# geoeo/ORB_SLAM3_V1.0

Measured on AMD Instinct MI355X. Metric: frames/sec ORB extract+match, 752x480 8-level 1000-feat; bit-exact kp/desc, higher is better.
Workload: dtype u8

## Files before the change

orb_slam3_v1.0_amd/csrc/kernels_match_proj.hip:

```cpp
#include <algorithm>
#include <cstdio>
#include <cstdlib>
#include <cstring>

#include "device_math.h"
#include "match_common.h"

#include "match_proj.h"

#pragma clang fp contract(off)

namespace orbfe {

using namespace proj;

namespace {


template <bool LDS, class KeyFn>
__device__ __forceinline__ void block_sort_keys(unsigned long long* sKeys, unsigned long long* gKeys, int n, int P, int tid, KeyFn keyOf)
{
    for (int j = tid; j < P; j += 1024) {
        const unsigned long long key = j < n ? keyOf(j) : ~0ull;
        if constexpr (LDS) sKeys[j] = key;
        else gKeys[j] = key;
    }
    __syncthreads();
    for (int k2 = 2; k2 <= P; k2 <<= 1) {
        for (int j2 = k2 >> 1; j2 > 0; j2 >>= 1) {
            for (int t = tid; t < (P >> 1); t += 1024) {
                const int lo = ((t & ~(j2 - 1)) << 1) | (t & (j2 - 1));
                const int hi = lo | j2;
                const bool up = (lo & k2) == 0;
                unsigned long long a, b;
                if constexpr (LDS) { a = sKeys[lo]; b = sKeys[hi]; }
                else { a = gKeys[lo]; b = gKeys[hi]; }
                if ((a > b) == up) {
                    if constexpr (LDS) { sKeys[lo] = b; sKeys[hi] = a; }
                    else { gKeys[lo] = b; gKeys[hi] = a; }
                }
            }
            __syncthreads();
        }
    }
}

template <class KeyFn>
__device__ __forceinline__ void block_sort_keys_reg(unsigned long long* sKeys, int n, int P, int tid, KeyFn keyOf)
{
    unsigned long long key = tid < n ? keyOf(tid) : ~0ull;
    int buf = 0;
    for (int k2 = 2; k2 <= P; k2 <<= 1) {
        for (int j2 = k2 >> 1; j2 > 0; j2 >>= 1) {
            unsigned long long other;
            if (j2 >= 64) {
                unsigned long long* b = sKeys + buf * 1024;
                b[tid] = key;
                __syncthreads();
                other = b[tid ^ j2];
                buf ^= 1;
            } else {
                other = shfl_xor_u64(key, j2);
            }
            const bool up = (tid & k2) == 0;
            const bool lower = (tid & j2) == 0;
            const unsigned long long mn = key < other ? key : other, mx = key < other ? other : key;
            key = (lower == up) ? mn : mx;
        }
    }
    __syncthreads();
    sKeys[tid] = key;
    __syncthreads();
}

constexpr int kCellBits = 22;

template <bool LDS>
__device__ __forceinline__ void proj_grid_body(const ProjArgs& A)
{
    __shared__ unsigned long long sKeys[LDS ? kSortLds : 1];
    __shared__ int sRankOf[LDS ? kSortLds : 1];
    const int f = blockIdx.x;
    const int tid = threadIdx.x;
    const int n = min(A.nKp[f], A.kpStride);
    const int nCells = A.g.cols * A.g.rows;
    const orbfe_keypoint* kp = A.kp + (size_t)f * A.kpStride;
    unsigned long long* gKeys = A.sortKeys + (size_t)f * A.sortCap;
    int* gRankOf = A.rankOf + (size_t)f * A.kpStride;
    int P = 1;
    while (P < n) P <<= 1;
    for (int j = tid; j < A.kpStride; j += 1024) A.matchOut[(size_t)f * A.kpStride + j] = -1;
    auto cellOf = [&](int j) {
        const orbfe_keypoint& k = kp[j];
        float px = k.x - A.g.minX;
        px = px * A.g.invW;
        float py = k.y - A.g.minY;
        py = py * A.g.invH;
        const int posX = (int)roundf(px), posY = (int)roundf(py);
        const int lin = posY * A.g.cols + posX;
        int v = nCells;
        if (lin >= 0 && lin < nCells) v = (lin % A.g.cols) * A.g.rows + lin / A.g.cols;
        return v;
    };
    auto key1 = [&](int j) { return ((unsigned long long)cellOf(j) << kRankBits) | (unsigned long long)j; };
    const bool regSort = LDS && P <= 1024;
    if (regSort) block_sort_keys_reg(sKeys, n, P, tid, key1);
    else block_sort_keys<LDS>(sKeys, gKeys, n, P, tid, key1);
    for (int r = tid; r < n; r += 1024) {
        unsigned long long key;
        if constexpr (LDS) key = sKeys[r];
        else key = gKeys[r];
        const int idx = (int)(key & kRankMask);
        A.order[(size_t)f * A.kpStride + r] = idx;
        A.octByRank[(size_t)f * A.kpStride + r] = (uint8_t)min(max(kp[idx].octave, 0), 31);
        if constexpr (LDS) sRankOf[idx] = r;
        else gRankOf[idx] = r;
    }
    __syncthreads();
    auto key2 = [&](int j) {
        const unsigned long long lvl = (unsigned long long)min(max(kp[j].octave, 0), 31);
        return (lvl << (kRankBits + kCellBits + 1)) | ((unsigned long long)cellOf(j) << kRankBits) | (unsigned long long)j;
    };
    if (regSort) block_sort_keys_reg(sKeys, n, P, tid, key2);
    else block_sort_keys<LDS>(sKeys, gKeys, n, P, tid, key2);
    const unsigned long long* desc = reinterpret_cast<const unsigned long long*>(A.desc + (size_t)f * A.kpStride * 32);
    for (int p = tid; p < n; p += 1024) {
        unsigned long long key;
        if constexpr (LDS) key = sKeys[p];
        else key = gKeys[p];
        const int idx = (int)(key & kRankMask);
        const int v = (int)((key >> kRankBits) & ((1u << (kCellBits + 1)) - 1u));
        const int lvl = (int)(key >> (kRankBits + kCellBits + 1));
        const orbfe_keypoint k = kp[idx];
        int rank;
        if constexpr (LDS) rank = sRankOf[idx];
        else rank = gRankOf[idx];
        const int cy = v < nCells ? v % A.g.rows : 0x7fff;
        A.rec[(size_t)f * A.kpStride + p] = make_int4(rank, lvl | (cy << 8), __float_as_int(k.x), __float_as_int(k.y));
        unsigned long long* dd = A.descS + ((size_t)f * A.kpStride + p) * 4;
        dd[0] = desc[(size_t)idx * 4 + 0];
        dd[1] = desc[(size_t)idx * 4 + 1];
        dd[2] = desc[(size_t)idx * 4 + 2];
        dd[3] = desc[(size_t)idx * 4 + 3];
    }
    const int tabStride = A.g.cols + 1;
    int* cs = A.colStart + (size_t)f * A.tabLevels * tabStride;
    const int nTab = A.tabLevels * tabStride;
    for (int e = tid; e < nTab; e += 1024) {
        const int l = e / tabStride;
        const int v = (e - l * tabStride) * A.g.rows;
        const unsigned long long want = ((unsigned long long)l << (kCellBits + 1)) | (unsigned long long)v;
        int lo = 0, hi = n;
        while (lo < hi) {
            const int mid = (lo + hi) >> 1;
            unsigned long long key;
            if constexpr (LDS) key = sKeys[mid];
            else key = gKeys[mid];
            if ((key >> kRankBits) < want) lo = mid + 1;
            else hi = mid;
        }
        cs[e] = lo;
    }
}

constexpr int kTilesX = 8, kTilesY = 6;
constexpr int kSortBuckets = 32 * kTilesX * kTilesY + 1;

__device__ __forceinline__ int sort_bucket(const ProjArgs& A, const orbfe_map_point& mp)
{
    const bool valid = mp.in_view && !(A.farPoints && mp.track_depth > A.thFar) && !mp.bad;
    if (!valid) return kSortBuckets - 1;
    const int lvl = min(max(mp.level, 0), 31);
    const int cx = (int)((mp.proj_x - A.g.minX) * A.g.invW), cy = (int)((mp.proj_y - A.g.minY) * A.g.invH);
    const int tx = min(max(cx * kTilesX / A.g.cols, 0), kTilesX - 1);
    const int ty = min(max(cy * kTilesY / A.g.rows, 0), kTilesY - 1);
    return (lvl * kTilesY + ty) * kTilesX + tx;
}

__device__ __forceinline__ void proj_sort_body(const ProjArgs& A)
{
    __shared__ int sHist[kSortBuckets];
    const int f = blockIdx.x;
    const int tid = threadIdx.x;
    for (int b = tid; b < kSortBuckets; b += 1024) sHist[b] = 0;
    __syncthreads();
    const orbfe_map_point* mps = A.mps + (size_t)f * A.M;
    for (int i = tid; i < A.M; i += 1024) atomicAdd(&sHist[sort_bucket(A, mps[i])], 1);
    __syncthreads();
    {
        static_assert(kSortBuckets <= 2048, "two buckets per thread");
        __shared__ int sWaveTot[16];
        const int b0 = 2 * tid, b1 = 2 * tid + 1;
        const int c0 = b0 < kSortBuckets ? sHist[b0] : 0, c1 = b1 < kSortBuckets ? sHist[b1] : 0;
        const int lane = tid & 63, wv = tid >> 6;
        int incl = c0 + c1;
#pragma unroll
        for (int d = 1; d < 64; d <<= 1) {
            const int o = __shfl_up(incl, d);
            if (lane >= d) incl += o;
        }
        if (lane == 63) sWaveTot[wv] = incl;
        __syncthreads();
        int base = incl - (c0 + c1);
        for (int q = 0; q < wv; q++) base += sWaveTot[q];
        if (b0 < kSortBuckets) sHist[b0] = base;
        if (b1 < kSortBuckets) sHist[b1] = base + c0;
    }
    __syncthreads();
    for (int i = tid; i < A.M; i += 1024) {
        const int pos = atomicAdd(&sHist[sort_bucket(A, mps[i])], 1);
        A.perm[(size_t)f * A.M + pos] = i;
    }
}

template <bool LDS, bool SORT_MPS>
__global__ __launch_bounds__(1024) void proj_prepare_kernel(ProjArgs A)
{
    if constexpr (SORT_MPS) {
        if (blockIdx.y == 1) {
            proj_sort_body(A);
            return;
        }
    }
    proj_grid_body<LDS>(A);
}

constexpr int kTopkLds = 768;

struct TopkLds {
    int4 rec[kTopkLds];
    unsigned long long desc[kTopkLds][4];
};

__device__ __forceinline__ void topk_insert_round(uint32_t (&keys)[kTopK], uint32_t (&pend)[kTopkPend])
{
    const uint32_t key = pend[0];
#pragma unroll
    for (int t = 0; t < kTopkPend - 1; t++) pend[t] = pend[t + 1];
    pend[kTopkPend - 1] = kKey32None;
#pragma unroll
    for (int t = kTopK - 1; t > 0; t--) keys[t] = umed3(keys[t - 1], key, keys[t]);
    keys[0] = min(keys[0], key);
}

template <bool LDS, bool WIDE>
__device__ __forceinline__ int topk_scan(const ProjArgs& A, const MpWindow& w, const int* cs, int tabStride, const int4* rec,
                                         const unsigned long long* descS, const TopkLds* S, int segBase,
                                         unsigned long long d0, unsigned long long d1, unsigned long long d2,
                                         unsigned long long d3, uint32_t (&keys)[kTopK])
{
    int total = 0;
    uint32_t pend[kTopkPend];
#pragma unroll
    for (int t = 0; t < kTopkPend; t++) pend[t] = kKey32None;
    const int lFirst = max(w.minLevel, 0), l1 = w.maxLevel;
    for (int l0 = lFirst; l0 <= (WIDE ? l1 : lFirst); l0 += 2) {
    int plo[2], phi[2];
#pragma unroll
    for (int k = 0; k < 2; k++) {
        const int l = min(l0 + k, l1);
        const int* csl = cs + (size_t)l * tabStride;
        plo[k] = csl[w.minCX];
        phi[k] = (l0 + k <= l1) ? csl[w.maxCX + 1] : plo[k];
    }
#pragma unroll
    for (int k = 0; k < 2; k++) {
        int4 qn = make_int4(0, 0, 0, 0);
        if (plo[k] < phi[k]) {
            if constexpr (LDS) qn = S->rec[plo[k] - segBase];
            else qn = rec[plo[k]];
        }
        for (int p = plo[k]; p < phi[k]; p++) {
            const int4 q = qn;
            if (p + 1 < phi[k]) {
                if constexpr (LDS) qn = S->rec[p + 1 - segBase];
                else qn = rec[p + 1];
            }
            const int cy = q.y >> 8;
            const float dx = __int_as_float(q.z) - w.x, dy = __int_as_float(q.w) - w.y;
            if (cy >= w.minCY && cy <= w.maxCY && fabsf(dx) < w.r && fabsf(dy) < w.r) {
                int dist;
                if constexpr (LDS) {
                    const unsigned long long* kd = S->desc[p - segBase];
                    dist = hamming256(kd, d0, d1, d2, d3);
                } else {
                    const unsigned long long* kd = descS + (size_t)p * 4;
                    dist = hamming256(kd, d0, d1, d2, d3);
                }
                if (dist < A.dCut) {
                    total++;
                    const uint32_t key = make_key32(dist, q.x);
                    if (key < keys[kTopK - 1]) {
#pragma unroll
                        for (int t = kTopkPend - 1; t > 0; t--) pend[t] = pend[t - 1];
                        pend[0] = key;
                    }
                }
            }
            if (__ballot(pend[kTopkPend - 1] != kKey32None)) topk_insert_round(keys, pend);
        }
    }
    }
    while (__ballot(pend[0] != kKey32None)) topk_insert_round(keys, pend);
    return total;
}

template <bool WIDE>
__global__ __launch_bounds__(256) void proj_topk_kernel(ProjArgs A)
{
    __shared__ TopkLds S;
    __shared__ int sLvlLo, sLvlHi;
    const int f = blockIdx.y;
    const int slotIdx = blockIdx.x * 256 + threadIdx.x;
    const bool live = slotIdx < A.M;
    const int i = live ? A.perm[(size_t)f * A.M + slotIdx] : 0;
    MpWindow w;
    w.valid = false;
    w.minLevel = w.maxLevel = 0;
    if (live) w = mp_window(A, A.mps[(size_t)f * A.M + i]);
    if (threadIdx.x == 0) { sLvlLo = 64; sLvlHi = -1; }
    __syncthreads();
    if (w.valid) {
        atomicMin(&sLvlLo, max(w.minLevel, 0));
        atomicMax(&sLvlHi, w.maxLevel);
    }
    __syncthreads();
    const int tabStride = A.g.cols + 1;
    const int* cs = A.colStart + (size_t)f * A.tabLevels * tabStride;
    const int4* rec = A.rec + (size_t)f * A.kpStride;
    const unsigned long long* descS = A.descS + (size_t)f * A.kpStride * 4;
    int segBase = 0, segEnd = 0;
    if (sLvlHi >= 0) {
        segBase = cs[(size_t)sLvlLo * tabStride];
        segEnd = sLvlHi + 1 < A.tabLevels ? cs[(size_t)(sLvlHi + 1) * tabStride] : min(A.nKp[f], A.kpStride);
    }
    const bool useLds = segEnd - segBase <= kTopkLds;
    if (useLds) {
        const int nSeg = segEnd - segBase;
        const uint4* gRec = reinterpret_cast<const uint4*>(rec + segBase);
        const uint4* gDesc = reinterpret_cast<const uint4*>(descS + (size_t)segBase * 4);
        uint4* lRec = reinterpret_cast<uint4*>(S.rec);
        uint4* lDesc = reinterpret_cast<uint4*>(&S.desc[0][0]);
        for (int j0 = 0; j0 < nSeg * 2; j0 += 4 * 256) {
            uint4 v[4];
#pragma unroll
            for (int k = 0; k < 4; k++) {
                const int j = j0 + k * 256 + (int)threadIdx.x;
                v[k] = make_uint4(0u, 0u, 0u, 0u);
                if (j < nSeg * 2) v[k] = gDesc[j];
            }
#pragma unroll
            for (int k = 0; k < 4; k++) {
                const int j = j0 + k * 256 + (int)threadIdx.x;
                if (j < nSeg * 2) lDesc[j] = v[k];
            }
        }
        for (int j0 = 0; j0 < nSeg; j0 += 4 * 256) {
            uint4 v[4];
#pragma unroll
            for (int k = 0; k < 4; k++) {
                const int j = j0 + k * 256 + (int)threadIdx.x;
                v[k] = make_uint4(0u, 0u, 0u, 0u);
                if (j < nSeg) v[k] = gRec[j];
            }
#pragma unroll
            for (int k = 0; k < 4; k++) {
                const int j = j0 + k * 256 + (int)threadIdx.x;
                if (j < nSeg) lRec[j] = v[k];
            }
        }
    }
    __syncthreads();
    if (!live) return;
    uint32_t keys[kTopK];
#pragma unroll
    for (int t = 0; t < kTopK; t++) keys[t] = kKey32None;
    int total = 0;
    if (w.valid) {
        const unsigned long long* dp = reinterpret_cast<const unsigned long long*>(A.mpDesc + ((size_t)f * A.M + i) * 32);
        const unsigned long long d0 = dp[0], d1 = dp[1], d2 = dp[2], d3 = dp[3];
        if (useLds) total = topk_scan<true, WIDE>(A, w, cs, tabStride, rec, descS, &S, segBase, d0, d1, d2, d3, keys);
        else total = topk_scan<false, WIDE>(A, w, cs, tabStride, rec, descS, &S, segBase, d0, d1, d2, d3, keys);
    }
    A.cnt[(size_t)f * A.M + i] = total;
    uint4* dst = reinterpret_cast<uint4*>(A.topk + ((size_t)f * A.M + i) * kTopK);
#pragma unroll
    for (int t = 0; t < kTopK / 4; t++) dst[t] = make_uint4(keys[4 * t], keys[4 * t + 1], keys[4 * t + 2], keys[4 * t + 3]);
}

constexpr int kWaveListCap = 128;

__device__ __forceinline__ void rank_emit_lds(const uint32_t* list, int n, int limit, uint32_t* out, int lane)
{
    const uint32_t e0 = lane < n ? list[lane] : kKey32None;
    const uint32_t e1 = lane + 64 < n ? list[lane + 64] : kKey32None;
    int r0 = 0, r1 = 0;
    for (int b = 0; b < n; b++) {
        const uint32_t kb = list[b];
        r0 += kb < e0;
        r1 += kb < e1;
    }
    __builtin_amdgcn_wave_barrier();
    if (lane < n && r0 < limit) out[r0] = e0;
    if (lane + 64 < n && r1 < limit) out[r1] = e1;
    asm volatile("s_waitcnt lgkmcnt(0)" ::: "memory");
    __builtin_amdgcn_wave_barrier();
}

template <bool WIDE, bool LDS>
__device__ __forceinline__ void topk_wave_body(const ProjArgs& A, const TopkLds& S, uint32_t (*sList)[2][kWaveListCap], int f, int lane,
                                               int wv, int nMine, int i, const MpWindow& w, const int* cs, int tabStride,
                                               const int4* rec, const unsigned long long* descS, int segBase)
{
    constexpr int NLV = WIDE ? 3 : 2;
    int plo[NLV], phi[NLV];
    {
        const int l0 = max(w.minLevel, 0), l1 = w.maxLevel;
#pragma unroll
        for (int k = 0; k < NLV; k++) {
            const int l = min(l0 + k, l1);
            const int* csl = cs + (size_t)l * tabStride;
            plo[k] = w.valid ? csl[w.minCX] : 0;
            phi[k] = (w.valid && l0 + k <= l1) ? csl[w.maxCX + 1] : plo[k];
        }
    }
    const int validI = w.valid ? 1 : 0;
    uint32_t dq[8] = {0, 0, 0, 0, 0, 0, 0, 0};
    if (w.valid) {
        const uint4* dp = reinterpret_cast<const uint4*>(A.mpDesc + ((size_t)f * A.M + i) * 32);
        const uint4 a = dp[0], b = dp[1];
        dq[0] = a.x; dq[1] = a.y; dq[2] = a.z; dq[3] = a.w; dq[4] = b.x; dq[5] = b.y; dq[6] = b.z; dq[7] = b.w;
    }
#pragma unroll
    for (int k = 0; k < NLV; k++) asm volatile("" : "+v"(plo[k]), "+v"(phi[k]));
#pragma unroll
    for (int k = 0; k < 8; k++) asm volatile("" : "+v"(dq[k]));
    {
        int iv = i;
        asm volatile("s_waitcnt vmcnt(0)" : "+v"(iv));
    }
    for (int j = 0; j < nMine; j++) {
        const int mp = __builtin_amdgcn_readlane(i, j);
        uint32_t* dst = A.topk + ((size_t)f * A.M + mp) * kTopK;
        int total = 0, listN = 0, cur = 0;
        if (__builtin_amdgcn_readlane(validI, j)) {
            const float x = __int_as_float(__builtin_amdgcn_readlane(__float_as_int(w.x), j));
            const float y = __int_as_float(__builtin_amdgcn_readlane(__float_as_int(w.y), j));
            const float r = __int_as_float(__builtin_amdgcn_readlane(__float_as_int(w.r), j));
            const int minCY = __builtin_amdgcn_readlane(w.minCY, j), maxCY = __builtin_amdgcn_readlane(w.maxCY, j);
            unsigned long long d[4];
#pragma unroll
            for (int k = 0; k < 4; k++)
                d[k] = (unsigned long long)(uint32_t)__builtin_amdgcn_readlane((int)dq[2 * k], j) |
                       ((unsigned long long)(uint32_t)__builtin_amdgcn_readlane((int)dq[2 * k + 1], j) << 32);
            int a[NLV], len[NLV], lenAll = 0;
#pragma unroll
            for (int k = 0; k < NLV; k++) {
                a[k] = __builtin_amdgcn_readlane(plo[k], j);
                len[k] = __builtin_amdgcn_readlane(phi[k], j) - a[k];
                lenAll += len[k];
            }
            for (int base = 0; base < lenAll; base += 64) {
                if (listN > 64) {
                    rank_emit_lds(sList[wv][cur], listN, 64, sList[wv][cur ^ 1], lane);
                    cur ^= 1;
                    listN = 64;
                }
                const int idx = base + lane;
                bool q = false;
                uint32_t key = kKey32None;
                if (idx < lenAll) {
                    int p = a[0] + idx;
                    if (idx >= len[0]) p = a[1] + (idx - len[0]);
                    if constexpr (NLV == 3)
                        if (idx >= len[0] + len[1]) p = a[2] + (idx - len[0] - len[1]);
                    int4 rq;
                    if constexpr (LDS) rq = S.rec[p - segBase];
                    else rq = rec[p];
                    const int cy = rq.y >> 8;
                    const float dx = __int_as_float(rq.z) - x, dy = __int_as_float(rq.w) - y;
                    if (cy >= minCY && cy <= maxCY && fabsf(dx) < r && fabsf(dy) < r) {
                        int dist;
                        if constexpr (LDS) {
                            const unsigned long long* kd = S.desc[p - segBase];
                            dist = hamming256(kd, d[0], d[1], d[2], d[3]);
                        } else {
                            const unsigned long long* kd = descS + (size_t)p * 4;
                            dist = hamming256(kd, d[0], d[1], d[2], d[3]);
                        }
                        if (dist < A.dCut) {
                            q = true;
                            key = make_key32(dist, rq.x);
                        }
                    }
                }
                const unsigned long long mask = __ballot(q);
                if (mask) {
                    if (q)
                        sList[wv][cur][listN + (int)__builtin_amdgcn_mbcnt_hi((uint32_t)(mask >> 32),
                                                                              __builtin_amdgcn_mbcnt_lo((uint32_t)mask, 0u))] = key;
                    const int c = __popcll(mask);
                    listN += c;
                    total += c;
                }
            }
            if (total) {
                asm volatile("s_waitcnt lgkmcnt(0)" ::: "memory");
                __builtin_amdgcn_wave_barrier();
                if (listN > 64) {
                    rank_emit_lds(sList[wv][cur], listN, 64, sList[wv][cur ^ 1], lane);
                    cur ^= 1;
                    listN = 64;
                }
                const uint32_t e = lane < listN ? sList[wv][cur][lane] : kKey32None;
                int rk = 0;
                for (int b = 0; b < listN; b++) rk += (uint32_t)__builtin_amdgcn_readlane((int)e, b) < e;
                if (lane < listN && rk < kTopK) dst[rk] = e;
                if (lane >= listN && lane < kTopK) dst[lane] = kKey32None;
            }
        }
        if (lane == 0) A.cnt[(size_t)f * A.M + mp] = total;
    }
}

template <bool WIDE>
__global__ __launch_bounds__(256) void proj_topk_wave_kernel(ProjArgs A, int mpw)
{
    __shared__ TopkLds S;
    __shared__ int sLvlLo, sLvlHi;
    __shared__ uint32_t sList[4][2][kWaveListCap];
    const int f = blockIdx.y;
    const int lane = threadIdx.x & 63;
    const int wv = __builtin_amdgcn_readfirstlane((int)(threadIdx.x >> 6));
    const int waveBase = (blockIdx.x * 4 + wv) * mpw;
    const int nMine = min(mpw, A.M - waveBase);
    const bool live = lane < nMine;
    const int i = live ? A.perm[(size_t)f * A.M + waveBase + lane] : 0;
    MpWindow w;
    w.valid = false;
    w.minLevel = w.maxLevel = 0;
    w.x = w.y = w.r = 0.0f;
    w.minCX = w.maxCX = w.minCY = w.maxCY = 0;
    if (live) w = mp_window(A, A.mps[(size_t)f * A.M + i]);
    if (threadIdx.x == 0) { sLvlLo = 64; sLvlHi = -1; }
    __syncthreads();
    if (w.valid) {
        atomicMin(&sLvlLo, max(w.minLevel, 0));
        atomicMax(&sLvlHi, w.maxLevel);
    }
    __syncthreads();
    const int tabStride = A.g.cols + 1;
    const int* cs = A.colStart + (size_t)f * A.tabLevels * tabStride;
    const int4* rec = A.rec + (size_t)f * A.kpStride;
    const unsigned long long* descS = A.descS + (size_t)f * A.kpStride * 4;
    int segBase = 0, segEnd = 0;
    if (sLvlHi >= 0) {
        segBase = cs[(size_t)sLvlLo * tabStride];
        segEnd = sLvlHi + 1 < A.tabLevels ? cs[(size_t)(sLvlHi + 1) * tabStride] : min(A.nKp[f], A.kpStride);
    }
    const bool useLds = segEnd - segBase <= kTopkLds;
    if (useLds) {
        const int nSeg = segEnd - segBase;
        const uint4* gRec = reinterpret_cast<const uint4*>(rec + segBase);
        const uint4* gDesc = reinterpret_cast<const uint4*>(descS + (size_t)segBase * 4);
        uint4* lRec = reinterpret_cast<uint4*>(S.rec);
        uint4* lDesc = reinterpret_cast<uint4*>(&S.desc[0][0]);
        for (int j0 = 0; j0 < nSeg * 2; j0 += 4 * 256) {
            uint4 v[4];
#pragma unroll
            for (int k = 0; k < 4; k++) {
                const int j = j0 + k * 256 + (int)threadIdx.x;
                if (j < nSeg * 2) v[k] = gDesc[j];
            }
#pragma unroll
            for (int k = 0; k < 4; k++) {
                const int j = j0 + k * 256 + (int)threadIdx.x;
                if (j < nSeg * 2) lDesc[j] = v[k];
            }
        }
        for (int j0 = 0; j0 < nSeg; j0 += 4 * 256) {
            uint4 v[4];
#pragma unroll
            for (int k = 0; k < 4; k++) {
                const int j = j0 + k * 256 + (int)threadIdx.x;
                if (j < nSeg) v[k] = gRec[j];
            }
#pragma unroll
            for (int k = 0; k < 4; k++) {
                const int j = j0 + k * 256 + (int)threadIdx.x;
                if (j < nSeg) lRec[j] = v[k];
            }
        }
    }
    __syncthreads();
    if (useLds) topk_wave_body<WIDE, true>(A, S, sList, f, lane, wv, nMine, i, w, cs, tabStride, rec, descS, segBase);
    else topk_wave_body<WIDE, false>(A, S, sList, f, lane, wv, nMine, i, w, cs, tabStride, rec, descS, segBase);
}

constexpr int kResN = 2048;

constexpr int kResNDesc = 1280;

template <int N, bool DESC, bool IMG>
struct ResolveLdsT {
    int claim[3][N];
    uint8_t oct[IMG ? N : 1];
    int4 rec[IMG ? N : 1];
    unsigned long long desc[DESC ? N * 4 : 4];
};

template <bool IMG, bool DESC, typename SLds>
__device__ __forceinline__ void full_scan_top2_wave(const ProjArgs& A, int f, int i, const MpWindow& w,
                                                    const unsigned long long (&d4)[4], const int* cs, const int* claim,
                                                    const SLds* S, int lane, uint32_t& k1, uint32_t& k2)
{
    k1 = kKey32None;
    k2 = kKey32None;
    if (w.valid) {
        const int tabStride = A.g.cols + 1;
        const int4* rec = A.rec + (size_t)f * A.kpStride;
        const unsigned long long* descS = A.descS + (size_t)f * A.kpStride * 4;
        for (int l = max(w.minLevel, 0); l <= w.maxLevel; l++) {
            const int* csl = cs + (size_t)l * tabStride;
            const int plo = csl[w.minCX], phi = csl[w.maxCX + 1];
            for (int p = plo + lane; p < phi; p += 64) {
                int4 q;
                if constexpr (IMG) q = S->rec[p];
                else q = rec[p];
                if (claim[q.x] < i) continue;
                const int cy = q.y >> 8;
                if (cy < w.minCY || cy > w.maxCY) continue;
                const float dx = __int_as_float(q.z) - w.x, dy = __int_as_float(q.w) - w.y;
                if (!(fabsf(dx) < w.r && fabsf(dy) < w.r)) continue;
                int dist;
                if constexpr (DESC) dist = hamming256(reinterpret_cast<const uint2*>(S->desc + (size_t)p * 4), d4);
                else dist = hamming256(reinterpret_cast<const uint2*>(descS + (size_t)p * 4), d4);
                if (dist >= A.dCut) continue;
                const uint32_t key = make_key32(dist, q.x);
                k2 = umed3(k1, key, k2);
                k1 = min(k1, key);
            }
        }
    }
    wave_top2_u32(k1, k2);
}

constexpr int kFbLds = 192;
constexpr int kResTabLds = 1024;
constexpr int kFbBatched = 32;

template <bool LDS, int THREADS, int N = kResN, bool DESC = false, bool IMG = LDS, int FB = kFbLds>
__global__ __launch_bounds__(THREADS) void proj_resolve_kernel(ProjArgs A)
{
    static_assert(LDS || !IMG, "the LDS image goes with LDS claim tables");
    __shared__ ResolveLdsT<N, DESC, IMG> S;
    __shared__ int sChanged[2];
    __shared__ int sGaveUp[2];
    __shared__ int sCount;
    __shared__ int sFbCount[2];
    __shared__ int sFbMp[THREADS];
    __shared__ uint32_t sFbK1[THREADS], sFbK2[THREADS];
    __shared__ MpWindow sFbWin[FB];
    __shared__ unsigned long long sFbDesc[FB][4];
    __shared__ int sTab[LDS ? kResTabLds : 1];
    const int f = blockIdx.x;
    const int tid = threadIdx.x;
    const int n = min(A.nKp[f], A.kpStride);
    const int M = A.M;
    int* Tfin = LDS ? S.claim[0] : A.claimG + ((size_t)f * 3 + 0) * A.kpStride;
    int* Tcur = LDS ? S.claim[1] : A.claimG + ((size_t)f * 3 + 1) * A.kpStride;
    int* Tnxt = LDS ? S.claim[2] : A.claimG + ((size_t)f * 3 + 2) * A.kpStride;
    const orbfe_map_point* mps = A.mps + (size_t)f * M;
    const int* order = A.order + (size_t)f * A.kpStride;
    const int4* rec = A.rec + (size_t)f * A.kpStride;
    const int* initObs = A.initObs ? A.initObs + (size_t)f * A.kpStride : nullptr;

    for (int r = tid; r < n; r += THREADS) {
        const int v = (initObs && initObs[order[r]] > 0) ? -1 : kClaimFree;
        Tfin[r] = v;
        Tcur[r] = v;
    }
    const uint8_t* octByRank = A.octByRank + (size_t)f * A.kpStride;
    if constexpr (IMG) {
        for (int r = tid; r < n; r += THREADS) {
            S.rec[r] = rec[r];
            S.oct[r] = octByRank[r];
        }
    }
    if constexpr (DESC) {
        const unsigned long long* dsrc = A.descS + (size_t)f * A.kpStride * 4;
        for (int q = tid; q < n * 4; q += THREADS) S.desc[q] = dsrc[q];
    }
    const int tabStride = A.g.cols + 1;
    const int* csG = A.colStart + (size_t)f * A.tabLevels * tabStride;
    const bool tabInLds = LDS && A.tabLevels * tabStride <= kResTabLds;
    if (tabInLds)
        for (int k = tid; k < A.tabLevels * tabStride; k += THREADS) sTab[k] = csG[k];
    const int* cs = tabInLds ? sTab : csG;
    if (tid == 0) sCount = 0;
    int nAccepted = 0;
    __syncthreads();

    for (int chunk = 0; chunk < M; chunk += THREADS) {
        const int i = chunk + tid;
        const bool live = i < M;
        int c = 0, obs = 0;
        uint32_t keys[kTopK];
#pragma unroll
        for (int t = 0; t < kTopK; t++) keys[t] = kKey32None;
        if (live) {
            c = A.cnt[(size_t)f * M + i];
            obs = mps[i].observations;
            if (c > 0) {
                const uint4* src = reinterpret_cast<const uint4*>(A.topk + ((size_t)f * M + i) * kTopK);
#pragma unroll
                for (int t = 0; t < kTopK / 4; t++) {
                    const uint4 q = src[t];
                    keys[4 * t] = q.x; keys[4 * t + 1] = q.y; keys[4 * t + 2] = q.z; keys[4 * t + 3] = q.w;
                }
            }
        }
        int res = -1;
        uint32_t k1 = kKey32None, k2 = kKey32None;
        bool k2StandIn = false;
        for (int iter = 0; iter <= THREADS + 1; iter++) {
            if (tid == 0) { sChanged[iter & 1] = 0; sFbCount[iter & 1] = 0; sGaveUp[iter & 1] = 0; }
            if (res >= 0 && obs > 0) atomicMin(&Tcur[res], i);
            __syncthreads();
            const int* claim = Tcur;
            bool look = iter == 0 || sGaveUp[(iter & 1) ^ 1] != 0;
            if (!look && c > 0) {
                const int c1 = k1 != kKey32None ? claim[(int)(k1 & kRankMask)] : kClaimFree;
                const int c2 = (k2 != kKey32None && !k2StandIn) ? claim[(int)(k2 & kRankMask)] : kClaimFree;
                look = c1 < i || c2 < i;
            }
            int slot = -1;
            if (c > 0 && look) {
                k1 = kKey32None;
                k2 = kKey32None;
                k2StandIn = false;
                int cl[kTopK];
#pragma unroll
                for (int t = 0; t < kTopK; t++) cl[t] = claim[keys[t] != kKey32None ? (int)(keys[t] & kRankMask) : 0];
#pragma unroll
                for (int t = 0; t < kTopK; t++) {
                    const uint32_t m = cl[t] >= i ? keys[t] : kKey32None;
                    k2 = umed3(k1, m, k2);
                    k1 = min(k1, m);
                }
                if (k2 == kKey32None && c > kTopK) {
                    const int dK = (int)(keys[kTopK - 1] >> kRankBits);
                    bool decided = false;
                    if (k1 == kKey32None) decided = dK > ORBFE_TH_HIGH;
                    else {
                        const int bd = (int)(k1 >> kRankBits);
                        decided = bd > ORBFE_TH_HIGH || (A.nnRatio > 0.f && !((float)bd > A.nnRatio * (float)dK));
                        if (decided) {
                            k2 = keys[kTopK - 1];
                            k2StandIn = true;
                        }
                    }
                    if (!decided) {
                        slot = atomicAdd(&sFbCount[iter & 1], 1);
                        sFbMp[slot] = i;
                        if (slot < FB) {
                            sFbWin[slot] = mp_window(A, mps[i]);
                            const unsigned long long* dp = reinterpret_cast<const unsigned long long*>(A.mpDesc + ((size_t)f * M + i) * 32);
#pragma unroll
                            for (int t = 0; t < 4; t++) sFbDesc[slot][t] = dp[t];
                        }
#ifdef ORBFE_DIAG
                        atomicAdd(&A.dbg[f * 4 + 1], 1);
                        if (slot >= FB) atomicAdd(&A.dbg[f * 4 + 2], 1);
#endif
                    }
                }
            }
            for (int k = tid; k < n; k += THREADS) Tnxt[k] = Tfin[k];
            auto verdict = [&]() {
                int result = -1;
                if (k1 != kKey32None) {
                    const int bestDist = (int)(k1 >> kRankBits), bestRank = (int)(k1 & kRankMask);
                    int bestLevel;
                    if constexpr (IMG) bestLevel = S.oct[bestRank];
                    else bestLevel = octByRank[bestRank];
                    int bestDist2 = 256, bestLevel2 = -1;
                    if (k2 != kKey32None) {
                        bestDist2 = (int)(k2 >> kRankBits);
                        const int r2 = (int)(k2 & kRankMask);
                        if constexpr (IMG) bestLevel2 = S.oct[r2];
                        else bestLevel2 = octByRank[r2];
                    }
                    if (bestDist <= ORBFE_TH_HIGH) {
                        const bool reject = bestLevel == bestLevel2 && (float)bestDist > A.nnRatio * (float)bestDist2;
                        if (!reject) result = bestRank;
                    }
                }
                return result;
            };
            auto move_to = [&](int result) {
                if (result != res) {
                    if (res >= 0 && obs > 0 && claim[res] == i) sGaveUp[iter & 1] = 1;
                    res = result;
                    sChanged[iter & 1] = 1;
                }
            };
            if (slot < 0 && look && c > 0) move_to(verdict());
            __syncthreads();
            if (sFbCount[iter & 1] > 0) {
                const int nFb = sFbCount[iter & 1];
                for (int q = __builtin_amdgcn_readfirstlane(tid >> 6); q < nFb; q += THREADS / 64) {
                    uint32_t a1, a2;
                    const int mp = sFbMp[q];
                    MpWindow w;
                    unsigned long long d4[4];
                    if (q < FB) {
                        w = sFbWin[q];
#pragma unroll
                        for (int t = 0; t < 4; t++) d4[t] = sFbDesc[q][t];
                    } else {
                        w = mp_window(A, mps[mp]);
                        const unsigned long long* dp = reinterpret_cast<const unsigned long long*>(A.mpDesc + ((size_t)f * M + mp) * 32);
#pragma unroll
                        for (int t = 0; t < 4; t++) d4[t] = dp[t];
                    }
                    full_scan_top2_wave<IMG, DESC>(A, f, mp, w, d4, cs, claim, &S, tid & 63, a1, a2);
                    if ((tid & 63) == 0) { sFbK1[q] = a1; sFbK2[q] = a2; }
                }
                __syncthreads();
                if (slot >= 0) {
                    k1 = sFbK1[slot];
                    k2 = sFbK2[slot];
                    move_to(verdict());
                }
                __syncthreads();
            }
#ifdef ORBFE_DIAG
            if (tid == 0) atomicAdd(&A.dbg[f * 4 + 0], 1);
#endif
            if (!sChanged[iter & 1]) break;
            int* const tq = Tcur;
            Tcur = Tnxt;
            Tnxt = tq;
        }
        {
            int* const tq = Tfin;
            Tfin = Tcur;
            Tcur = tq;
        }
        if (chunk + THREADS < M) {
            for (int k = tid; k < n; k += THREADS) Tcur[k] = Tfin[k];
            __syncthreads();
        }
        if (res >= 0) {
            atomicMax(&A.matchOut[(size_t)f * A.kpStride + order[res]], i);
            nAccepted++;
        }
    }
    if (nAccepted) atomicAdd(&sCount, nAccepted);
    __syncthreads();
    if (tid == 0) A.nMatches[f] = sCount;
}

}

namespace proj {

void proj_prepare_launch(hipStream_t s, const ProjArgs& A, bool sortMps)
{
    const bool lds = A.kpStride <= kSortLds;
    if (sortMps) {
        if (lds) hipLaunchKernelGGL((proj_prepare_kernel<true, true>), dim3(A.B, 2), dim3(1024), 0, s, A);
        else hipLaunchKernelGGL((proj_prepare_kernel<false, true>), dim3(A.B, 2), dim3(1024), 0, s, A);
    } else {
        if (lds) hipLaunchKernelGGL((proj_prepare_kernel<true, false>), dim3(A.B), dim3(1024), 0, s, A);
        else hipLaunchKernelGGL((proj_prepare_kernel<false, false>), dim3(A.B), dim3(1024), 0, s, A);
    }
}

int proj_dcut(float nnRatio)
{
    int D = 256;
    for (int d = 0; d < 256; d++)
        if (!((float)ORBFE_TH_HIGH > nnRatio * (float)d)) {
            D = d;
            break;
        }
    return std::max(D, ORBFE_TH_HIGH + 1);
}

int proj_setup(MatchScratch& m, ProjArgs& A, Carver sc, size_t hostNeed, std::string& err, size_t* endOff)
{
    const int B = A.B, M = A.M;
    A.sortCap = 1;
    while (A.sortCap < A.kpStride) A.sortCap <<= 1;
    const bool ldsSort = A.kpStride <= kSortLds;
    const size_t oKeys = sc.take(ldsSort ? 8 : (size_t)B * A.sortCap * sizeof(unsigned long long));
    A.tabLevels = std::min(std::max(A.nLevels, 1), 32);
    A.dCut = proj_dcut(A.nnRatio);
    const size_t oOrder = sc.take((size_t)B * A.kpStride * sizeof(int));
    const size_t oOct = sc.take((size_t)B * A.kpStride);
    const size_t oRankOf = sc.take(ldsSort ? 8 : (size_t)B * A.kpStride * sizeof(int));
    const size_t oRec = sc.take((size_t)B * A.kpStride * sizeof(int4));
    const size_t oDescS = sc.take((size_t)B * A.kpStride * 32);
    const size_t oCol = sc.take((size_t)B * A.tabLevels * ((size_t)A.g.cols + 1) * sizeof(int));
    const size_t oCnt = sc.take((size_t)B * std::max(M, 1) * sizeof(int));
    const size_t oTopk = sc.take((size_t)B * kTopK * std::max(M, 1) * sizeof(uint32_t));
    const size_t oClaim = sc.take((size_t)B * 3 * A.kpStride * sizeof(int));
    const size_t oPerm = sc.take((size_t)B * std::max(M, 1) * sizeof(int));
    const size_t oDbg = sc.take((size_t)B * 4 * sizeof(int));
    if (endOff) *endOff = sc.off;
    int rc = ensure(m, sc.off, hostNeed + 256, err);
    if (rc != ORBFE_OK) return rc;
    uint8_t* dp = static_cast<uint8_t*>(m.d);
    A.sortKeys = reinterpret_cast<unsigned long long*>(dp + oKeys);
    A.order = reinterpret_cast<int*>(dp + oOrder);
    A.octByRank = dp + oOct;
    A.rankOf = reinterpret_cast<int*>(dp + oRankOf);
    A.rec = reinterpret_cast<int4*>(dp + oRec);
    A.descS = reinterpret_cast<unsigned long long*>(dp + oDescS);
    A.colStart = reinterpret_cast<int*>(dp + oCol);
    A.cnt = reinterpret_cast<int*>(dp + oCnt);
    A.topk = reinterpret_cast<uint32_t*>(dp + oTopk);
    A.claimG = reinterpret_cast<int*>(dp + oClaim);
    A.perm = reinterpret_cast<int*>(dp + oPerm);
    A.dbg = reinterpret_cast<int*>(dp + oDbg);
    return ORBFE_OK;
}

int proj_launch(hipStream_t s, ProjArgs& A, std::string& err)
{
    if (A.M == 0) {
        proj_prepare_launch(s, A, false);
        MCHK(hipMemsetAsync(A.nMatches, 0, (size_t)A.B * sizeof(int), s));
        return ORBFE_OK;
    }
#ifdef ORBFE_DIAG
    MCHK(hipMemsetAsync(A.dbg, 0, (size_t)A.B * 4 * sizeof(int), s));
#endif
    proj_prepare_launch(s, A, true);
    const int blocks256 = (A.M + 255) / 256;
    if ((long long)blocks256 * A.B >= 128) {
        if (A.mode == kModeReloc)
            hipLaunchKernelGGL(proj_topk_kernel<true>, dim3(blocks256, A.B), dim3(256), 0, s, A);
        else
            hipLaunchKernelGGL(proj_topk_kernel<false>, dim3(blocks256, A.B), dim3(256), 0, s, A);
    } else {
        int mpw = 64;
        while (mpw > 1 && (long long)((A.M + 4 * mpw - 1) / (4 * mpw)) * A.B < 512) mpw >>= 1;
        const dim3 grid((A.M + 4 * mpw - 1) / (4 * mpw), A.B);
        if (A.mode == kModeReloc)
            hipLaunchKernelGGL(proj_topk_wave_kernel<true>, grid, dim3(256), 0, s, A, mpw);
        else
            hipLaunchKernelGGL(proj_topk_wave_kernel<false>, grid, dim3(256), 0, s, A, mpw);
    }
    const bool lds = A.kpStride <= kResN;
    const bool batched = A.B >= kResolveBatchedMinFrames;
#ifdef ORBFE_DIAG
    static const int envT = getenv("ORBFE_RESOLVE_THREADS") ? atoi(getenv("ORBFE_RESOLVE_THREADS")) : -1;
    const int rt = envT >= 0 ? envT : (batched ? 0 : kResolveThreads);
#else
    const int rt = batched ? 0 : kResolveThreads;
#endif
    if (rt == 0) {
        if (lds) hipLaunchKernelGGL((proj_resolve_kernel<true, 256, kResN, false, false, kFbBatched>), dim3(A.B), dim3(256), 0, s, A);
        else hipLaunchKernelGGL((proj_resolve_kernel<false, 256, kResN, false, false, kFbBatched>), dim3(A.B), dim3(256), 0, s, A);
    } else if (lds && A.kpStride <= kResNDesc && rt == kResolveThreads) {
        hipLaunchKernelGGL((proj_resolve_kernel<true, kResolveThreads, kResNDesc, true>), dim3(A.B), dim3(kResolveThreads), 0, s, A);
    } else if (rt == 256) {
        if (lds) hipLaunchKernelGGL((proj_resolve_kernel<true, 256>), dim3(A.B), dim3(256), 0, s, A);
        else hipLaunchKernelGGL((proj_resolve_kernel<false, 256>), dim3(A.B), dim3(256), 0, s, A);
    } else {
        if (lds) hipLaunchKernelGGL((proj_resolve_kernel<true, kResolveThreads>), dim3(A.B), dim3(kResolveThreads), 0, s, A);
        else hipLaunchKernelGGL((proj_resolve_kernel<false, kResolveThreads>), dim3(A.B), dim3(kResolveThreads), 0, s, A);
    }
    MCHK(hipGetLastError());
    return ORBFE_OK;
}

}

void match_scratch_free(MatchScratch& m)
{
    if (m.d) (void)hipFree(m.d);
    if (m.hpin) (void)hipHostFree(m.hpin);
    m = MatchScratch();
}

int match_projection_run(MatchScratch& m, hipStream_t s, const orbfe_frame_view* F, int M, const orbfe_map_point* mps,
                         const uint8_t* mpDesc, const int* initObs, float th, int farPoints, float thFar,
                         float nnRatio, int* matchOut, int* nMatches, std::string& err)
{
    const int n = F->n;
    for (int i = 0; i < n; i++) matchOut[i] = -1;
    *nMatches = 0;
    if (n == 0 || M == 0) return ORBFE_OK;
    if (n >= (1 << 20) || F->grid_cols > 65535 || F->grid_rows > 32767 || F->n_levels < 1 ||
        (long long)F->grid_cols * F->grid_rows > kMaxCells)
        return ORBFE_ERR_UNSUPPORTED;
    for (int i = 0; i < M; i++)
        if (mps[i].in_view && (mps[i].level < 0 || mps[i].level >= F->n_levels)) return ORBFE_ERR_INVALID_ARG;

    Carver in;
    const size_t oKp = in.take((size_t)n * sizeof(orbfe_keypoint));
    const size_t oDesc = in.take((size_t)n * 32);
    const size_t oMp = in.take((size_t)M * sizeof(orbfe_map_point));
    const size_t oMpDesc = in.take((size_t)M * 32);
    const size_t oObs = in.take((size_t)n * sizeof(int));
    const size_t oSf = in.take((size_t)F->n_levels * sizeof(float));
    const size_t oN = in.take(sizeof(int));
    const size_t oMatch = in.take((size_t)n * sizeof(int));
    const size_t oNM = in.take(sizeof(int));
    const size_t inBytes = in.off;
    const size_t hostNeed = inBytes + (size_t)n * sizeof(int) + 64;

    ProjArgs A{};
    A.B = 1; A.M = M; A.kpStride = n;
    A.g = GridDesc{F->grid_cols, F->grid_rows, F->min_x, F->min_y, F->grid_inv_w, F->grid_inv_h};
    A.th = th; A.thFar = thFar; A.nnRatio = nnRatio; A.farPoints = farPoints; A.bFactor = th != 1.0;
    A.nLevels = F->n_levels;
    int rc = proj_setup(m, A, in, hostNeed, err);
    if (rc != ORBFE_OK) return rc;
    uint8_t* hp = static_cast<uint8_t*>(m.hpin);
    uint8_t* dp = static_cast<uint8_t*>(m.d);
    memcpy(hp + oKp, F->kp, (size_t)n * sizeof(orbfe_keypoint));
    memcpy(hp + oDesc, F->desc, (size_t)n * 32);
    memcpy(hp + oMp, mps, (size_t)M * sizeof(orbfe_map_point));
    memcpy(hp + oMpDesc, mpDesc, (size_t)M * 32);
    if (initObs) memcpy(hp + oObs, initObs, (size_t)n * sizeof(int));
    memcpy(hp + oSf, F->scale_factors, (size_t)F->n_levels * sizeof(float));
    memcpy(hp + oN, &n, sizeof(int));
    MCHK(hipMemcpyAsync(dp, hp, oMatch, hipMemcpyHostToDevice, s));
    A.kp = reinterpret_cast<const orbfe_keypoint*>(dp + oKp);
    A.desc = dp + oDesc;
    A.nKp = reinterpret_cast<const int*>(dp + oN);
    A.mps = reinterpret_cast<const orbfe_map_point*>(dp + oMp);
    A.mpDesc = dp + oMpDesc;
    A.initObs = initObs ? reinterpret_cast<const int*>(dp + oObs) : nullptr;
    A.scaleFactors = reinterpret_cast<const float*>(dp + oSf);
    A.matchOut = reinterpret_cast<int*>(dp + oMatch);
    A.nMatches = reinterpret_cast<int*>(dp + oNM);
    int* hNM = reinterpret_cast<int*>(hp + inBytes);
    int* hMatch = hNM + 2;
    rc = proj_launch(s, A, err);
    if (rc != ORBFE_OK) return rc;
    MCHK(hipMemcpyAsync(hMatch, A.matchOut, (size_t)n * sizeof(int), hipMemcpyDeviceToHost, s));
    MCHK(hipMemcpyAsync(hNM, A.nMatches, sizeof(int), hipMemcpyDeviceToHost, s));
    MCHK(hipStreamSynchronize(s));
#ifdef ORBFE_DIAG
    if (getenv("ORBFE_DEBUG_MATCH")) {
        int dbg[4] = {0, 0, 0, 0};
        (void)copy_sync(dbg, A.dbg, sizeof dbg, hipMemcpyDeviceToHost, s);
        fprintf(stderr, "[orbfe] match_projection: n=%d M=%d sweeps=%d cooperative_rescans=%d unparked_rescans=%d\n", n, M, dbg[0], dbg[1],
                dbg[2]);
    }
#endif
    memcpy(matchOut, hMatch, (size_t)n * sizeof(int));
    *nMatches = *hNM;
    return ORBFE_OK;
}

int match_projection_batch_device(MatchScratch& m, hipStream_t s, int B, const orbfe_keypoint* dKp, const uint8_t* dDesc,
                                  const int* dN, int kpStride, int gridCols, int gridRows, float minX, float minY,
                                  float invW, float invH, const float* dScaleFactors, int nLevels, int M,
                                  const orbfe_map_point* dMps, const uint8_t* dMpDesc, const int* dInitObs, float th,
                                  int farPoints, float thFar, float nnRatio, int* dMatchOut, int* dNMatches,
                                  std::string& err)
{
    if (kpStride >= (1 << 20) || gridCols > 65535 || gridRows > 32767 || (long long)gridCols * gridRows > kMaxCells)
        return ORBFE_ERR_UNSUPPORTED;
    ProjArgs A{};
    A.B = B; A.M = M; A.kpStride = kpStride;
    A.g = GridDesc{gridCols, gridRows, minX, minY, invW, invH};
    A.th = th; A.thFar = thFar; A.nnRatio = nnRatio; A.farPoints = farPoints; A.bFactor = th != 1.0;
    A.kp = dKp; A.desc = dDesc; A.nKp = dN; A.mps = dMps; A.mpDesc = dMpDesc; A.initObs = dInitObs;
    A.scaleFactors = dScaleFactors; A.nLevels = nLevels;
    A.matchOut = dMatchOut;
    A.nMatches = dNMatches;
    int rc = proj_setup(m, A, Carver(), 64, err);
    if (rc != ORBFE_OK) return rc;
    return proj_launch(s, A, err);
}

}
```

Measured before the change: 227,400.

## Replace second bitonic sort with stable level counting-sort in projection prepare

In the LDS path, the second full bitonic sort by (level, cell, index) is replaced with a stable per-level counting sort built from the cell-sorted keys. It uses wave ballots for ranks within a level, per-chunk level counts and a block exclusive scan. Rank is then read directly by slot instead of through an inverse-rank table. The change also templates the kernel on thread count, adding a 256-thread variant with four keys per thread, but that variant is only reachable through a diagnostic environment variable. The scan code is factored into a shared helper.

```diff
diff --git a/orb_slam3_v1.0_amd/csrc/kernels_match_proj.hip b/orb_slam3_v1.0_amd/csrc/kernels_match_proj.hip
--- a/orb_slam3_v1.0_amd/csrc/kernels_match_proj.hip
+++ b/orb_slam3_v1.0_amd/csrc/kernels_match_proj.hip
@@ -17,10 +17,10 @@
 namespace {
 
 
-template <bool LDS, class KeyFn>
+template <bool LDS, int NT, class KeyFn>
 __device__ __forceinline__ void block_sort_keys(unsigned long long* sKeys, unsigned long long* gKeys, int n, int P, int tid, KeyFn keyOf)
 {
-    for (int j = tid; j < P; j += 1024) {
+    for (int j = tid; j < P; j += NT) {
         const unsigned long long key = j < n ? keyOf(j) : ~0ull;
         if constexpr (LDS) sKeys[j] = key;
         else gKeys[j] = key;
@@ -28,7 +28,7 @@
     __syncthreads();
     for (int k2 = 2; k2 <= P; k2 <<= 1) {
         for (int j2 = k2 >> 1; j2 > 0; j2 >>= 1) {
-            for (int t = tid; t < (P >> 1); t += 1024) {
+            for (int t = tid; t < (P >> 1); t += NT) {
                 const int lo = ((t & ~(j2 - 1)) << 1) | (t & (j2 - 1));
                 const int hi = lo | j2;
                 const bool up = (lo & k2) == 0;
@@ -73,13 +73,104 @@
     __syncthreads();
 }
 
+template <class KeyFn>
+__device__ __forceinline__ void block_sort_keys_reg4(unsigned long long* sKeys, int n, int P, int tid, KeyFn keyOf)
+{
+    unsigned long long key[4];
+#pragma unroll
+    for (int q = 0; q < 4; q++) key[q] = q * 256 + tid < n ? keyOf(q * 256 + tid) : ~0ull;
+    const int Q = P > 512 ? 4 : (P > 256 ? 2 : 1);
+    auto cx = [](unsigned long long& a, unsigned long long& b, bool up) {
+        const unsigned long long mn = a < b ? a : b, mx = a < b ? b : a;
+        a = up ? mn : mx;
+        b = up ? mx : mn;
+    };
+    int buf = 0;
+    for (int k2 = 2; k2 <= P; k2 <<= 1) {
+        for (int j2 = k2 >> 1; j2 > 0; j2 >>= 1) {
+            if (j2 == 512) {
+                cx(key[0], key[2], true);
+                cx(key[1], key[3], true);
+                continue;
+            }
+            if (j2 == 256) {
+                cx(key[0], key[1], true);
+                if (Q == 4) cx(key[2], key[3], k2 == 1024);
+                continue;
+            }
+            unsigned long long other[4];
+            if (j2 >= 64) {
+                unsigned long long* b = sKeys + buf * 1024;
+#pragma unroll
+                for (int q = 0; q < 4; q++)
+                    if (q < Q) b[q * 256 + tid] = key[q];
+                __syncthreads();
+#pragma unroll
+                for (int q = 0; q < 4; q++)
+                    if (q < Q) other[q] = b[(q * 256 + tid) ^ j2];
+                buf ^= 1;
+            } else {
+#pragma unroll
+                for (int q = 0; q < 4; q++)
+                    if (q < Q) other[q] = shfl_xor_u64(key[q], j2);
+            }
+            const bool lower = (tid & j2) == 0;
+#pragma unroll
+            for (int q = 0; q < 4; q++)
+                if (q < Q) {
+                    const bool up = ((q * 256 + tid) & k2) == 0;
+                    const unsigned long long mn = key[q] < other[q] ? key[q] : other[q], mx = key[q] < other[q] ? other[q] : key[q];
+                    key[q] = (lower == up) ? mn : mx;
+                }
+        }
+    }
+    __syncthreads();
+#pragma unroll
+    for (int q = 0; q < 4; q++)
+        if (q < Q) sKeys[q * 256 + tid] = key[q];
+    __syncthreads();
+}
+
+template <int NT, int PER>
+__device__ __forceinline__ void block_excl_scan(int* s, int count, int* sWaveTot, int tid)
+{
+    int c[PER];
+    int sum = 0;
+#pragma unroll
+    for (int q = 0; q < PER; q++) {
+        c[q] = PER * tid + q < count ? s[PER * tid + q] : 0;
+        sum += c[q];
+    }
+    const int lane = tid & 63, wv = tid >> 6;
+    int incl = sum;
+#pragma unroll
+    for (int d = 1; d < 64; d <<= 1) {
+        const int o = __shfl_up(incl, d);
+        if (lane >= d) incl += o;
+    }
+    if (lane == 63) sWaveTot[wv] = incl;
+    __syncthreads();
+    int base = incl - sum;
+    for (int q = 0; q < wv; q++) base += sWaveTot[q];
+#pragma unroll
+    for (int q = 0; q < PER; q++) {
+        if (PER * tid + q < count) s[PER * tid + q] = base;
+        base += c[q];
+    }
+}
+
 constexpr int kCellBits = 22;
 
-template <bool LDS>
+constexpr int kLvlChunks = kSortLds / 64;
+
+template <bool LDS, int NT>
 __device__ __forceinline__ void proj_grid_body(const ProjArgs& A)
 {
+    constexpr bool ONE = LDS;
     __shared__ unsigned long long sKeys[LDS ? kSortLds : 1];
     __shared__ int sRankOf[LDS ? kSortLds : 1];
+    __shared__ int sLvlCnt[ONE ? 32 * kLvlChunks : 1];
+    __shared__ int sLvlTot[ONE ? NT / 64 : 1];
     const int f = blockIdx.x;
     const int tid = threadIdx.x;
     const int n = min(A.nKp[f], A.kpStride);
@@ -89,7 +180,17 @@
     int* gRankOf = A.rankOf + (size_t)f * A.kpStride;
     int P = 1;
     while (P < n) P <<= 1;
-    for (int j = tid; j < A.kpStride; j += 1024) A.matchOut[(size_t)f * A.kpStride + j] = -1;
+    for (int j = tid; j < A.kpStride; j += NT) A.matchOut[(size_t)f * A.kpStride + j] = -1;
+    if constexpr (ONE)
+        for (int e = tid; e < 32 * kLvlChunks; e += NT) sLvlCnt[e] = 0;
+    auto sortKeys = [&](auto keyOf) {
+        if (LDS && P <= 1024) {
+            if constexpr (NT == 1024) block_sort_keys_reg(sKeys, n, P, tid, keyOf);
+            else block_sort_keys_reg4(sKeys, n, P, tid, keyOf);
+        } else {
+            block_sort_keys<LDS, NT>(sKeys, gKeys, n, P, tid, keyOf);
+        }
+    };
     auto cellOf = [&](int j) {
         const orbfe_keypoint& k = kp[j];
         float px = k.x - A.g.minX;
@@ -103,28 +204,73 @@
         return v;
     };
     auto key1 = [&](int j) { return ((unsigned long long)cellOf(j) << kRankBits) | (unsigned long long)j; };
-    const bool regSort = LDS && P <= 1024;
-    if (regSort) block_sort_keys_reg(sKeys, n, P, tid, key1);
-    else block_sort_keys<LDS>(sKeys, gKeys, n, P, tid, key1);
-    for (int r = tid; r < n; r += 1024) {
-        unsigned long long key;
-        if constexpr (LDS) key = sKeys[r];
-        else key = gKeys[r];
-        const int idx = (int)(key & kRankMask);
-        A.order[(size_t)f * A.kpStride + r] = idx;
-        A.octByRank[(size_t)f * A.kpStride + r] = (uint8_t)min(max(kp[idx].octave, 0), 31);
-        if constexpr (LDS) sRankOf[idx] = r;
-        else gRankOf[idx] = r;
-    }
-    __syncthreads();
-    auto key2 = [&](int j) {
-        const unsigned long long lvl = (unsigned long long)min(max(kp[j].octave, 0), 31);
-        return (lvl << (kRankBits + kCellBits + 1)) | ((unsigned long long)cellOf(j) << kRankBits) | (unsigned long long)j;
-    };
-    if (regSort) block_sort_keys_reg(sKeys, n, P, tid, key2);
-    else block_sort_keys<LDS>(sKeys, gKeys, n, P, tid, key2);
+    sortKeys(key1);
+    if constexpr (ONE) {
+        constexpr int ITER = kSortLds / NT;
+        const int lane = tid & 63;
+        unsigned long long skey[ITER];
+        int pre[ITER];
+#pragma unroll
+        for (int it = 0; it < ITER; it++) {
+            pre[it] = 0;
+            skey[it] = 0;
+            if (it * NT < n) {
+                const int r = it * NT + tid;
+                const bool valid = r < n;
+                int lvl = 0;
+                if (valid) {
+                    const unsigned long long key = sKeys[r];
+                    const int idx = (int)(key & kRankMask);
+                    lvl = min(max(kp[idx].octave, 0), 31);
+                    A.order[(size_t)f * A.kpStride + r] = idx;
+                    A.octByRank[(size_t)f * A.kpStride + r] = (uint8_t)lvl;
+                    skey[it] = ((unsigned long long)lvl << (kRankBits + kCellBits + 1)) | key;
+                }
+                unsigned long long rem = __ballot(valid);
+                while (rem) {
+                    const int L = __builtin_amdgcn_readlane(lvl, __builtin_ctzll(rem));
+                    const unsigned long long m = __ballot(valid && lvl == L);
+                    if (valid && lvl == L)
+                        pre[it] = (int)__builtin_amdgcn_mbcnt_hi((uint32_t)(m >> 32), __builtin_amdgcn_mbcnt_lo((uint32_t)m, 0u));
+                    if (lane == 0) sLvlCnt[L * kLvlChunks + (r >> 6)] = __popcll(m);
+                    rem &= ~m;
+                }
+            }
+        }
+        __syncthreads();
+        block_excl_scan<NT, 32 * kLvlChunks / NT>(sLvlCnt, 32 * kLvlChunks, sLvlTot, tid);
+        __syncthreads();
+#pragma unroll
+        for (int it = 0; it < ITER; it++) {
+            const int r = it * NT + tid;
+            if (r < n) {
+                const int lvl = (int)(skey[it] >> (kRankBits + kCellBits + 1));
+                const int slot = sLvlCnt[lvl * kLvlChunks + (r >> 6)] + pre[it];
+                sKeys[slot] = skey[it];
+                sRankOf[slot] = r;
+            }
+        }
+        __syncthreads();
+    } else {
+        for (int r = tid; r < n; r += NT) {
+            unsigned long long key;
+            if constexpr (LDS) key = sKeys[r];
+            else key = gKeys[r];
+            const int idx = (int)(key & kRankMask);
+            A.order[(size_t)f * A.kpStride + r] = idx;
+            A.octByRank[(size_t)f * A.kpStride + r] = (uint8_t)min(max(kp[idx].octave, 0), 31);
+            if constexpr (LDS) sRankOf[idx] = r;
+            else gRankOf[idx] = r;
+        }
+        __syncthreads();
+        auto key2 = [&](int j) {
+            const unsigned long long lvl = (unsigned long long)min(max(kp[j].octave, 0), 31);
+            return (lvl << (kRankBits + kCellBits + 1)) | ((unsigned long long)cellOf(j) << kRankBits) | (unsigned long long)j;
+        };
+        sortKeys(key2);
+    }
     const unsigned long long* desc = reinterpret_cast<const unsigned long long*>(A.desc + (size_t)f * A.kpStride * 32);
-    for (int p = tid; p < n; p += 1024) {
+    for (int p = tid; p < n; p += NT) {
         unsigned long long key;
         if constexpr (LDS) key = sKeys[p];
         else key = gKeys[p];
@@ -133,7 +279,8 @@
         const int lvl = (int)(key >> (kRankBits + kCellBits + 1));
         const orbfe_keypoint k = kp[idx];
         int rank;
-        if constexpr (LDS) rank = sRankOf[idx];
+        if constexpr (ONE) rank = sRankOf[p];
+        else if constexpr (LDS) rank = sRankOf[idx];
         else rank = gRankOf[idx];
         const int cy = v < nCells ? v % A.g.rows : 0x7fff;
         A.rec[(size_t)f * A.kpStride + p] = make_int4(rank, lvl | (cy << 8), __float_as_int(k.x), __float_as_int(k.y));
@@ -146,7 +293,7 @@
     const int tabStride = A.g.cols + 1;
     int* cs = A.colStart + (size_t)f * A.tabLevels * tabStride;
     const int nTab = A.tabLevels * tabStride;
-    for (int e = tid; e < nTab; e += 1024) {
+    for (int e = tid; e < nTab; e += NT) {
         const int l = e / tabStride;
         const int v = (e - l * tabStride) * A.g.rows;
         const unsigned long long want = ((unsigned long long)l << (kCellBits + 1)) | (unsigned long long)v;
@@ -177,52 +324,37 @@
     return (lvl * kTilesY + ty) * kTilesX + tx;
 }
 
+template <int NT>
 __device__ __forceinline__ void proj_sort_body(const ProjArgs& A)
 {
     __shared__ int sHist[kSortBuckets];
+    __shared__ int sWaveTot[NT / 64];
     const int f = blockIdx.x;
     const int tid = threadIdx.x;
-    for (int b = tid; b < kSortBuckets; b += 1024) sHist[b] = 0;
+    for (int b = tid; b < kSortBuckets; b += NT) sHist[b] = 0;
     __syncthreads();
     const orbfe_map_point* mps = A.mps + (size_t)f * A.M;
-    for (int i = tid; i < A.M; i += 1024) atomicAdd(&sHist[sort_bucket(A, mps[i])], 1);
-    __syncthreads();
-    {
-        static_assert(kSortBuckets <= 2048, "two buckets per thread");
-        __shared__ int sWaveTot[16];
-        const int b0 = 2 * tid, b1 = 2 * tid + 1;
-        const int c0 = b0 < kSortBuckets ? sHist[b0] : 0, c1 = b1 < kSortBuckets ? sHist[b1] : 0;
-        const int lane = tid & 63, wv = tid >> 6;
-        int incl = c0 + c1;
-#pragma unroll
-        for (int d = 1; d < 64; d <<= 1) {
-            const int o = __shfl_up(incl, d);
-            if (lane >= d) incl += o;
-        }
-        if (lane == 63) sWaveTot[wv] = incl;
-        __syncthreads();
-        int base = incl - (c0 + c1);
-        for (int q = 0; q < wv; q++) base += sWaveTot[q];
-        if (b0 < kSortBuckets) sHist[b0] = base;
-        if (b1 < kSortBuckets) sHist[b1] = base + c0;
-    }
-    __syncthreads();
-    for (int i = tid; i < A.M; i += 1024) {
+    for (int i = tid; i < A.M; i += NT) atomicAdd(&sHist[sort_bucket(A, mps[i])], 1);
+    __syncthreads();
+    block_excl_scan<NT, (kSortBuckets + NT - 1) / NT>(sHist, kSortBuckets, sWaveTot, tid);
+    __syncthreads();
+    for (int i = tid; i < A.M; i += NT) {
         const int pos = atomicAdd(&sHist[sort_bucket(A, mps[i])], 1);
         A.perm[(size_t)f * A.M + pos] = i;
     }
 }
 
-template <bool LDS, bool SORT_MPS>
-__global__ __launch_bounds__(1024) void proj_prepare_kernel(ProjArgs A)
-{
+template <bool LDS, bool SORT_MPS, int NT>
+__global__ __launch_bounds__(NT) void proj_prepare_kernel(ProjArgs A)
+{
+    static_assert(NT == 1024 || NT == 256, "register sorts: one key per thread of 1024, four per thread of 256");
     if constexpr (SORT_MPS) {
         if (blockIdx.y == 1) {
-            proj_sort_body(A);
+            proj_sort_body<NT>(A);
             return;
         }
     }
-    proj_grid_body<LDS>(A);
+    proj_grid_body<LDS, NT>(A);
 }
 
 constexpr int kTopkLds = 768;
@@ -866,16 +998,26 @@
 
 namespace proj {
 
+template <bool SORT_MPS, int NT>
+static void prepare_launch_form(hipStream_t s, const ProjArgs& A)
+{
+    const dim3 grid(A.B, SORT_MPS ? 2 : 1);
+    if (A.kpStride <= kSortLds) hipLaunchKernelGGL((proj_prepare_kernel<true, SORT_MPS, NT>), grid, dim3(NT), 0, s, A);
+    else hipLaunchKernelGGL((proj_prepare_kernel<false, SORT_MPS, NT>), grid, dim3(NT), 0, s, A);
+}
+
 void proj_prepare_launch(hipStream_t s, const ProjArgs& A, bool sortMps)
 {
-    const bool lds = A.kpStride <= kSortLds;
-    if (sortMps) {
-        if (lds) hipLaunchKernelGGL((proj_prepare_kernel<true, true>), dim3(A.B, 2), dim3(1024), 0, s, A);
-        else hipLaunchKernelGGL((proj_prepare_kernel<false, true>), dim3(A.B, 2), dim3(1024), 0, s, A);
-    } else {
-        if (lds) hipLaunchKernelGGL((proj_prepare_kernel<true, false>), dim3(A.B), dim3(1024), 0, s, A);
-        else hipLaunchKernelGGL((proj_prepare_kernel<false, false>), dim3(A.B), dim3(1024), 0, s, A);
-    }
+#ifdef ORBFE_DIAG
+    static const int envT = getenv("ORBFE_PREPARE_THREADS") ? atoi(getenv("ORBFE_PREPARE_THREADS")) : -1;
+    if (envT == 0) {
+        if (sortMps) prepare_launch_form<true, 256>(s, A);
+        else prepare_launch_form<false, 256>(s, A);
+        return;
+    }
+#endif
+    if (sortMps) prepare_launch_form<true, 1024>(s, A);
+    else prepare_launch_form<false, 1024>(s, A);
 }
 
 int proj_dcut(float nnRatio)
```

Measured after the change: 228,400, median of 6. No clear change (+0.4%).
